# winddori2002/DEX-TTS

Measured on AMD Instinct MI355X. Metric: mel-frames/s at n_timesteps=50, 80-ch mel (sampler only); RTF, higher is better.
Workload: dtype bf16; 1 GPU; gedex_b1: gedex_lj B=1/GPU T=512 n_timesteps=50 (BASELINE.json configs[1]); global_batch=1, frames=512, hipgraph=False, parallelism=1 GPU

## Files before the change

dex_tts_amd/csrc/dex_api.hip:

```cpp
#include <hip/hip_runtime.h>
#include <cstdlib>

#include <cmath>
#include <cstdarg>
#include <atomic>
#include <cstdio>
#include <mutex>
#include <cstring>
#include <map>
#include <unordered_map>
#include <string_view>
#include <string>
#include <vector>

#include "../../include/dex_amd.h"
#include "kernels.h"
#include "weight_store.h"

using namespace dex;

namespace dex {
namespace {
const char* const KNOB_NAMES[] = {
    "DEX_CONV_STREAM", "DEX_CONV_PP", "DEX_CONV_SKIP_DEAD", "DEX_H_BF16", "DEX_ATTN_SEPARATE", "DEX_ATTN_Q64", "DEX_ATTN_Q64_TAIL", "DEX_ATTN_Q64_HALF", "DEX_DIT_XCDS", "DEX_ATTN_GENERIC", "DEX_RES2", "DEX_LP_INTER", "DEX_DIT_CHAIN",
    "DEX_DIT_CLUSTER", "DEX_DIT_CLUSTER_LOCAL", "DEX_ATTN_X_LP", "DEX_RES_X_LP", "DEX_CAT_LP", "DEX_XCD_MAP", "DEX_DEBUG_DROP_HANDOFF", "DEX_PATCH_FUSED",
    "DEX_CONV_DOWN", "DEX_CONVT_UP", "DEX_DEBUG_PLAN",
    "DEX_ATTN_SHARED_W8", "DEX_CONVT_MT", "DEX_CONVT_WGS", "DEX_CONV_DOWN_WGS", "DEX_CONV_REGW", "DEX_CONV_REGW_RES", "DEX_CONV_SMALL_MAX", "DEX_CONV_TH8",
    "DEX_CONV_W8", "DEX_DWCONV_CAP", "DEX_FINAL_CAP", "DEX_FIRST_CAP", "DEX_FIRST_MFMA", "DEX_GEMM_NWALK", "DEX_NWALK_SPLIT", "DEX_NWALK_BM", "DEX_POS_COL", "DEX_POS_COL_MIN",
    "DEX_POS_CT", "DEX_REGW_MIN_TILES", "DEX_REGW_WGS", "DEX_ROWCHAIN64", "DEX_ROWCHAIN64A", "DEX_TIV_CAP", "DEX_TV_CHAIN", "DEX_TIV_FOLD", "DEX_LINATTN_NSUB", "DEX_TV_FOLD", "DEX_OUT2_MIN", "DEX_NWALK_DMA",
    "DEX_LINATTN_HEADWAVES", "DEX_LINATTN_OUT2_HW", "DEX_CONV_ROUND1", "DEX_CONV_RESIDENT"};
constexpr int N_KNOBS = (int)(sizeof(KNOB_NAMES) / sizeof(KNOB_NAMES[0]));
int knob_parse(const char* e) {
    if (!e) return KNOB_UNSET;
    char* end = nullptr;
    const long v = strtol(e, &end, 10);
    if (end == e) {
        static bool warned = false;
        if (!warned) { warned = true; fprintf(stderr, "libdexamd: ignoring a DEX_* knob whose value '%s' is not an integer\n", e); }
        return KNOB_UNSET;
    }
// ... 1013 lines not shown
        DwConvP dw{};
        dw.X = X.p + X.coff; dw.ldx = X.ld; dw.xb = (long)P.Hm * P.Wm * X.ld; dw.Hi = P.Hm; dw.Wi = P.Wm; dw.C = mid;
        dw.k = c.dit_patch; dw.s = c.dit_stride; dw.pad = c.dit_patch / 2; dw.Wd = x->pe_dw; dw.bd = x->pe_db;
        dw.mask = mask_input ? mask : nullptr; dw.mask_ws = mask_ws; dw.mask_bstride = P.d.T;
        dw.Y = P.pe0; dw.Hf = P.Hf; dw.Wt = P.Wt; dw.B = B; dw.aff = in_aff;
        if (patch_fused()) {
            run("patch_embed", 2.0 * B * N * mid * (c.dit_patch * c.dit_patch + hid), 4.0 * B * (P.Hm * P.Wm * mid + N * hid),
                [&] { launch_patch_embed_fused(dw, x->pe_pw.nk[x->lpi()].p, x->pe_pb, P.emb, hid, x->precision, st); });
        } else {
            run("patch_dwconv_silu", 2.0 * B * N * mid * c.dit_patch * c.dit_patch, 4.0 * B * (P.Hm * P.Wm + N) * mid, [&] { launch_dwconv_silu(dw, st); });
            IGemmP pe = base_gemm(P.pe0, mid, 0, P.Hf, P.Wt, mid, x->pe_pw, hid, x->pe_pb, P.emb, hid, 0);
            gemm("patch_pointwise", pe);
        }
        const int G = c.dit_conv_pos_groups, kp = c.dit_conv_pos, cg = hid / G;
        int nsplit = POS_SPLIT, pcg = 0, pcgp = 0;
        if (x->lp() && x->pos_w.frag[x->lpi()].p) {
            PosConvP pcd{P.emb, x->pos_w.frag[x->lpi()].p, P.pos_part, P.Hf, P.Wt, hid, G, B};
            run("pos_conv", 2.0 * B * N * (double)kp * kp * cg * hid, 8.0 * B * N * hid + 2.0 * kp * kp * cg * hid, [&] { launch_pos_conv_direct(pcd, x->precision, st); });
            nsplit = 1;
        } else {
            const int cgp = (cg % 32) ? 64 : cg;
            const float* src = P.emb;
            if (cgp != cg) {
                run("pos_group_pad", 0, 8.0 * B * N * hid, [&] { launch_group_pad(P.emb, P.emb_pad, (long)B * N, G, cg, cgp, st); });
                src = P.emb_pad;
            }
            IGemmP pc = base_gemm(src, G * cgp, 0, P.Hf, P.Wt, cgp, x->pos_w, cgp, nullptr, P.pos_part, G * cgp, 0);
            pc.KH = kp; pc.KW = kp; pc.off_h = -(kp / 2); pc.off_w = -(kp / 2); pc.K = kp * kp * cgp;
            pc.groups = G; pc.w_gstride = (long)kp * kp * cgp * cgp; pc.ksplit = POS_SPLIT; pc.c_sstride = (long)B * N * G * cgp;
            gemm("pos_conv", pc);
            pcg = cgp != cg ? cg : 0; pcgp = cgp;
        }
        PosFinishP pf{P.pos_part, nsplit, (long)B * N * (pcg ? G * pcgp : hid), x->pos_b, P.emb, x->freq_pos, P.tok, P.Hf, P.Wt, hid, B, pcg, pcgp};
        run("pos_finish", 20.0 * B * N * hid, 4.0 * B * N * hid * (nsplit + 2), [&] { launch_pos_finish(pf, st); });
        if (debug) hipMemcpyAsync(P.dbg_tok, P.tok, (size_t)B * N * hid * 4, hipMemcpyDeviceToDevice, st);
        tap("tok_in", P.dbg_tok, (long)B * N, hid, hid);
        const float scale = 1.0f / sqrtf((float)(hid / c.dit_heads));
        const bool chain = x->lp() && dit_rowchain_supported(hid, mh) && c.dit_heads == 2 &&
                           !knob_off("DEX_DIT_CHAIN");
        for (int k = 0; k < c.dit_depth; ++k) {
            const DitBlockW& w = x->blocks[k];
            const float* ada = P.ada[k];
            const bool fuse_ln = x->lp() && ln_fusable(hid);
            DitChainP ch{};
            if (chain) {
                ch.ksplit = 0; ch.heads = c.dit_heads; ch.rows_per_batch = N; ch.X = P.tok; ch.ada = ada; ch.step = sp; ch.row_bstride = rbs; ch.M = B * N; ch.B = B;
                ch.Qh = (k & 1) ? P.qh : P.qh2; ch.Kh = (k & 1) ? P.kh : P.kh2; ch.Vt = (k & 1) ? P.vt : P.vt2;
                ch.Qin = (k & 1) ? P.qh2 : P.qh; ch.Kin = (k & 1) ? P.kh2 : P.kh; ch.Vin = (k & 1) ? P.vt2 : P.vt;
                ch.Npad = P.Npad;
// ... 100 lines not shown
                hipMemcpyAsync(dst, P.tok, (size_t)B * N * hid * 4, hipMemcpyDeviceToDevice, st);
                char nm[32]; snprintf(nm, sizeof nm, "tok_blk%d", k);
                tap(nm, dst, (long)B * N, hid, hid);
            }
        }
        const bool fuse_lnf = x->lp() && ln_fusable(hid);
        if (!fuse_lnf) {
            LnModP lf{P.tok, P.xn, N, hid, P.fin_mod, P.fin_mod + hid, 2L * hid, sp, B, rbs};
            run("ln_modulate", 8.0 * B * N * hid, 8.0 * B * N * hid, [&] { launch_ln_mod(lf, st); });
        }
        IGemmP fl = final_gemm(mask_ws, out, ldo, ocoff);
        if (cat_lp) { fl.C = reinterpret_cast<float*>(P.cat16); fl.c_lp = x->lp_kind(); }
        gemm("dit_final_unpatchify", fl);
    }

    bool patch_fused() const {
        const DexConfig& c = x->cfg;
        return x->lp() && !debug && !knob_off("DEX_PATCH_FUSED") &&
               patch_embed_fused_supported(c.dit_patch, mid_dim(c), c.dit_hidden, (long)P.d.B * P.N);
    }
    bool tiv_fold() const { return !debug && P.tiv_aff && knob_or("DEX_TIV_FOLD", 1) != 0; }
    bool tv_chain_on() const {
        return x->lp() && x->tv_wl.nk[x->lpi()].p && P.tv_kp && tv_chain_form(P.Hm * P.Wm, mid_dim(x->cfg), P.d.B);
    }
    bool tv_fold_on() const { return tv_chain_on() && x->lpi() != 2 && P.tv_G && knob_or("DEX_TV_FOLD", 1) != 0; }
    void dex_adaptors(const TD& X, int mask_ws) {
        const DexConfig& c = x->cfg;
        const int B = P.d.B, mid = mid_dim(c);
        const long npix = (long)P.Hm * P.Wm;
        InStatsP is{X.p + X.coff, X.ld, npix * X.ld, (int)npix, mid, P.tv_stats, B, mask, mask_ws, (long)P.d.T, P.Wm};
// ... 707 lines not shown
```

dex_tts_amd/csrc/kernels.h:

```cpp
#pragma once
#include <hip/hip_runtime.h>
#include <stdint.h>

namespace dex {

constexpr int KNOB_UNSET = -2147483647 - 1;
int knob(const char* name);
inline int knob_or(const char* name, int dflt) { const int v = knob(name); return v == KNOB_UNSET ? dflt : v; }
inline bool knob_off(const char* name) { return knob(name) == 0; }
inline bool knob_set(const char* name) { return knob(name) != KNOB_UNSET; }
inline int device_cus() {
    static const int n = [] { int dev = 0, v = 0; (void)hipGetDevice(&dev); (void)hipDeviceGetAttribute(&v, hipDeviceAttributeMultiprocessorCount, dev); return v > 0 ? v : 256; }();
    return n;
}

constexpr int GN_SLOTS = 32;
typedef long long gnfix_t;

extern thread_local const char* g_last_symbol;

constexpr int PREC_FP32 = 0, PREC_BF16 = 1, PREC_FP16 = 2, PREC_FP16X2 = 3;
inline bool prec_wsplit(int precision) { return precision == PREC_FP16X2; }
extern thread_local bool g_lp_wsplit;
inline bool prec_is_lp(int precision) { return precision != PREC_FP32; }
// ... 170 lines not shown
bool linattn_out2_lp_out_supported(int npix, int B);
bool linattn_fused_supported(int C);

struct DwConvP { const float* X; int ldx; long xb; int Hi, Wi, C; int k, s, pad; const float* Wd; const float* bd;
                 const float* mask; int mask_ws; long mask_bstride;
                 float* Y; int Hf, Wt; int B;
                 const float* aff = nullptr; };
void launch_dwconv_silu(const DwConvP& p, hipStream_t st);
bool patch_embed_fused_supported(int k, int C, int hid, long ntok);
void launch_patch_embed_fused(const DwConvP& p, const void* Wb, const float* bias, float* emb, int hid, int precision, hipStream_t st);

struct PosConvP { const float* X; const void* Wf; float* Y; int Hf, Wt, hid, G, B;
                  int ncol; };
bool pos_conv_direct_supported(int hid, int groups, int kernel, int Hf);
void launch_pos_conv_direct(const PosConvP& p, int precision, hipStream_t st);
struct PosFinishP { const float* part; int nsplit; long split_stride; const float* bias; const float* emb;
                    const float* freq_pos; float* tok; int Hf, Wt, D; int B;
                    int cg, cg_pad; };
void launch_pos_finish(const PosFinishP& p, hipStream_t st);
void launch_group_pad(const float* src, float* dst, long rows, int G, int cg, int cg_pad, hipStream_t st);

struct LnModP { const float* X; float* Y; int rows_per_batch; int D; const float* shift; const float* scale;
                long step_stride; int step; int B; int row_bstride = 0; };
void launch_ln_mod(const LnModP& p, hipStream_t st);

struct DitChainP { const float* O; int ksplit; long o_sstride; const float* ml; int heads; int rows_per_batch;
                   float* X; const void *Wp, *W1, *W2, *Wq; const float *bp, *b1, *b2, *bq;
                   const float* ada;
                   const float *next_shift, *next_scale; long next_step_stride;
                   void *Qh, *Kh, *Vt; int Npad; float qscale;
// ... 170 lines not shown
```

dex_tts_amd/csrc/kernels_lp.h:

```cpp
#include "kernels.h"
#include "lp_config.h"

namespace dex {
namespace DEX_LP_NS {

bool conv3x3_bf16_supported(int Cin, int Cout);
bool conv3x3_bf16_tail_supported(int C);
bool conv3x3_bf16_res_supported(int Cin, int Cout);
bool conv3x3_bf16_xb_supported(int Cin, int Cout);
void launch_conv3x3_lp(const Conv3P& p, hipStream_t st);
int conv3x3_stream_tiles(const Conv3P& p);
void launch_conv3x3_stream(const Conv3P& p, int tiles_per_wg, hipStream_t st);
bool conv3x3_regw_form(const Conv3P& p);
void launch_conv3x3_regw(const Conv3P& p, hipStream_t st);
bool linattn_out2_lp_out_supported(int npix, int B);
bool linattn_fused_supported(int C);
bool conv3x3_plain_lp_in_supported(int H, int W, int B, int Cin, int Cout);
bool conv3x3_res2_form(int H, int W, int B);
void launch_igemm_lp(const IGemmP& p, hipStream_t st);
bool attention_lp_shared_form(int Nq, int heads, int B, int ksplit);
bool igemm_nwalk_form(const IGemmP& p);
bool conv3x3_cat_lp_in_supported(int H, int W, int B, int Cin, int Cout);
bool convt_up_supported(int C, int H, int W, int ldx, int ldy);
void launch_convt_up(const ConvTUpP& p, hipStream_t st);
// ... 14 lines not shown
bool dit_rowchain_supported(int hidden, int mlp_hidden);
bool dit_rowchain64_form(int rows_per_batch, int B, int attn_inline);
bool dit_rowchain_cluster_form(int rows_per_batch, int B);
bool dit_rowchain_cluster_local_fits(int rows_per_batch, int B);
int dit_rowchain_cluster_xcds(int rows_per_batch, int B);
void launch_dit_rowchain(const DitChainP& p, hipStream_t st);
void launch_pack_lp_frag(const float* src, void* dst, int K, int N, hipStream_t st);
void launch_pack_lp_frag_nk(const float* src, void* dst, int K, int N, hipStream_t st);
void launch_linattn_kvctx(const LinKvCtxP& p, hipStream_t st);
void launch_linattn_merge(const LinMergeP& p, hipStream_t st);
void launch_linattn_out2(const LinOut2P& p, hipStream_t st);
bool patch_embed_fused_supported(int k, int C, int hid, long ntok);
void launch_patch_embed_fused(const DwConvP& p, const void* Wb, const float* bias, float* emb, int hid, hipStream_t st);
bool pos_conv_direct_supported(int hid, int groups, int kernel, int Hf);
void launch_pos_conv_direct(const PosConvP& p, hipStream_t st);

}
}
```

dex_tts_amd/csrc/lp_dispatch.hip:

```cpp
#include "kernels.h"

#include "kernels_lp.h"
#undef DEX_LP_NS
#define DEX_LP_NS f16
#include "kernels_lp.h"
#undef DEX_LP_NS
#define DEX_LP_NS f16w
#include "kernels_lp.h"
#undef DEX_LP_NS

namespace dex {

thread_local const char* g_last_symbol = nullptr;
thread_local bool g_lp_wsplit = false;

bool conv3x3_bf16_supported(int Cin, int Cout) { return (g_lp_wsplit ? f16w::conv3x3_bf16_supported(Cin, Cout) : bf16::conv3x3_bf16_supported(Cin, Cout)); }
bool conv3x3_bf16_tail_supported(int C) { return (g_lp_wsplit ? f16w::conv3x3_bf16_tail_supported(C) : bf16::conv3x3_bf16_tail_supported(C)); }
bool conv3x3_bf16_res_supported(int Cin, int Cout) { return (g_lp_wsplit ? f16w::conv3x3_bf16_res_supported(Cin, Cout) : bf16::conv3x3_bf16_res_supported(Cin, Cout)); }
bool conv3x3_bf16_xb_supported(int Cin, int Cout) { return (g_lp_wsplit ? f16w::conv3x3_bf16_xb_supported(Cin, Cout) : bf16::conv3x3_bf16_xb_supported(Cin, Cout)); }
bool conv3x3_plain_lp_in_supported(int H, int W, int B, int Cin, int Cout) { return (g_lp_wsplit ? f16w::conv3x3_plain_lp_in_supported(H, W, B, Cin, Cout) : bf16::conv3x3_plain_lp_in_supported(H, W, B, Cin, Cout)); }
bool linattn_out2_lp_out_supported(int npix, int B) { return (g_lp_wsplit ? f16w::linattn_out2_lp_out_supported(npix, B) : bf16::linattn_out2_lp_out_supported(npix, B)); }
bool linattn_fused_supported(int C) { return (g_lp_wsplit ? f16w::linattn_fused_supported(C) : bf16::linattn_fused_supported(C)); }
bool conv3x3_res2_form(int H, int W, int B) { return (g_lp_wsplit ? f16w::conv3x3_res2_form(H, W, B) : bf16::conv3x3_res2_form(H, W, B)); }
bool attention_lp_shared_form(int Nq, int heads, int B, int ksplit) { return (g_lp_wsplit ? f16w::attention_lp_shared_form(Nq, heads, B, ksplit) : bf16::attention_lp_shared_form(Nq, heads, B, ksplit)); }
bool igemm_nwalk_form(const IGemmP& p) { return (g_lp_wsplit ? f16w::igemm_nwalk_form(p) : bf16::igemm_nwalk_form(p)); }
bool conv3x3_cat_lp_in_supported(int H, int W, int B, int Cin, int Cout) { return (g_lp_wsplit ? f16w::conv3x3_cat_lp_in_supported(H, W, B, Cin, Cout) : bf16::conv3x3_cat_lp_in_supported(H, W, B, Cin, Cout)); }
bool conv3x3_strip_form(const Conv3P& p) { return (g_lp_wsplit ? f16w::conv3x3_stream_tiles(p) : bf16::conv3x3_stream_tiles(p)) != 0 || (g_lp_wsplit ? f16w::conv3x3_regw_form(p) : bf16::conv3x3_regw_form(p)); }
bool pos_conv_direct_supported(int hid, int groups, int kernel, int Hf) { return (g_lp_wsplit ? f16w::pos_conv_direct_supported(hid, groups, kernel, Hf) : bf16::pos_conv_direct_supported(hid, groups, kernel, Hf)); }
bool tv_chain_form(int npix, int C, int B) { return (g_lp_wsplit ? f16w::tv_chain_form(npix, C, B) : bf16::tv_chain_form(npix, C, B)); }
bool attention_direct_batch_regime(int N, int B) { return (g_lp_wsplit ? f16w::attention_direct_batch_regime(N, B) : bf16::attention_direct_batch_regime(N, B)); }
int attention_direct_ksplit(int N, int B) { return (g_lp_wsplit ? f16w::attention_direct_ksplit(N, B) : bf16::attention_direct_ksplit(N, B)); }
int attention_q64_ksplit(int N, int B, int max_split) { return (g_lp_wsplit ? f16w::attention_q64_ksplit(N, B, max_split) : bf16::attention_q64_ksplit(N, B, max_split)); }
void attention_q64_plan(int N, int B, int max_split, int* ks, int* tail_g, int* tail_ks) { (g_lp_wsplit ? f16w::attention_q64_plan(N, B, max_split, ks, tail_g, tail_ks) : bf16::attention_q64_plan(N, B, max_split, ks, tail_g, tail_ks)); }
bool conv_down_supported(int C, int H, int W, int ldx, int ldy, int x_coff) { return (g_lp_wsplit ? f16w::conv_down_supported(C, H, W, ldx, ldy, x_coff) : bf16::conv_down_supported(C, H, W, ldx, ldy, x_coff)); }
bool convt_up_supported(int C, int H, int W, int ldx, int ldy) { return (g_lp_wsplit ? f16w::convt_up_supported(C, H, W, ldx, ldy) : bf16::convt_up_supported(C, H, W, ldx, ldy)); }
bool patch_embed_fused_supported(int k, int C, int hid, long ntok) { return (g_lp_wsplit ? f16w::patch_embed_fused_supported(k, C, hid, ntok) : bf16::patch_embed_fused_supported(k, C, hid, ntok)); }
bool dit_rowchain_supported(int hidden, int mlp_hidden) { return (g_lp_wsplit ? f16w::dit_rowchain_supported(hidden, mlp_hidden) : bf16::dit_rowchain_supported(hidden, mlp_hidden)); }
bool dit_rowchain64_form(int rows_per_batch, int B, int attn_inline) { return (g_lp_wsplit ? f16w::dit_rowchain64_form(rows_per_batch, B, attn_inline) : bf16::dit_rowchain64_form(rows_per_batch, B, attn_inline)); }
bool dit_rowchain_cluster_form(int rows_per_batch, int B) { return (g_lp_wsplit ? f16w::dit_rowchain_cluster_form(rows_per_batch, B) : bf16::dit_rowchain_cluster_form(rows_per_batch, B)); }
int dit_rowchain_cluster_xcds(int rows_per_batch, int B) { return bf16::dit_rowchain_cluster_xcds(rows_per_batch, B); }
bool dit_rowchain_cluster_local_fits(int rows_per_batch, int B) { return (g_lp_wsplit ? f16w::dit_rowchain_cluster_local_fits(rows_per_batch, B) : bf16::dit_rowchain_cluster_local_fits(rows_per_batch, B)); }

#define DEX_LP_CALL(fn, ...) do { if (precision == PREC_FP16X2) f16w::fn(__VA_ARGS__); else if (precision == PREC_FP16) f16::fn(__VA_ARGS__); else bf16::fn(__VA_ARGS__); } while (0)
// ... 4 lines not shown
void launch_conv_down(const ConvDownP& p, int precision, hipStream_t st) { DEX_LP_CALL(launch_conv_down, p, st); }
void launch_attention_lp(const AttnP& p, int precision, hipStream_t st) { DEX_LP_CALL(launch_attention_lp, p, st); }
void launch_tv_kv_prep(const TvKvPrepP& p, int precision, hipStream_t st) { DEX_LP_CALL(launch_tv_kv_prep, p, st); }
void launch_tv_vfrag_prep(const TvKvPrepP& p, int precision, hipStream_t st) { DEX_LP_CALL(launch_tv_vfrag_prep, p, st); }
void launch_tv_chain(const TvChainP& p, int precision, hipStream_t st) { DEX_LP_CALL(launch_tv_chain, p, st); }
void launch_attention_direct(const AttnDirectP& p, int precision, hipStream_t st) { DEX_LP_CALL(launch_attention_direct, p, st); }
bool attention_q64_half_plan(int N, int B, int* half_g, int* half_n) { return bf16::attention_q64_half_plan(N, B, half_g, half_n); }
void launch_attention_q64(const AttnDirectP& p, int precision, hipStream_t st) { DEX_LP_CALL(launch_attention_q64, p, st); }
void launch_dit_rowchain(const DitChainP& p, int precision, hipStream_t st) { DEX_LP_CALL(launch_dit_rowchain, p, st); }
void launch_pack_lp_frag(const float* src, void* dst, int K, int N, int precision, hipStream_t st) { DEX_LP_CALL(launch_pack_lp_frag, src, dst, K, N, st); }
void launch_pack_lp_frag_nk(const float* src, void* dst, int K, int N, int precision, hipStream_t st) { DEX_LP_CALL(launch_pack_lp_frag_nk, src, dst, K, N, st); }
void launch_linattn_kvctx(const LinKvCtxP& p, int precision, hipStream_t st) { DEX_LP_CALL(launch_linattn_kvctx, p, st); }
void launch_linattn_merge(const LinMergeP& p, int precision, hipStream_t st) { DEX_LP_CALL(launch_linattn_merge, p, st); }
void launch_linattn_out2(const LinOut2P& p, int precision, hipStream_t st) { DEX_LP_CALL(launch_linattn_out2, p, st); }
void launch_pos_conv_direct(const PosConvP& p, int precision, hipStream_t st) { DEX_LP_CALL(launch_pos_conv_direct, p, st); }
void launch_patch_embed_fused(const DwConvP& p, const void* Wb, const float* bias, float* emb, int hid, int precision, hipStream_t st) { DEX_LP_CALL(launch_patch_embed_fused, p, Wb, bias, emb, hid, st); }

}
```

dex_tts_amd/csrc/patch_embed.hip:

```cpp
#include <hip/hip_runtime.h>
#include "kernels.h"
#include "lp_util.h"
#include "kernels_lp.h"

namespace dex {
namespace DEX_LP_NS {

typedef float f32x16 __attribute__((ext_vector_type(16)));
typedef unsigned short u16;

namespace {
constexpr int PE_TOK = 8;
__device__ __forceinline__ float silu_pe(float x) { return x * __builtin_amdgcn_rcpf(1.f + __expf(-x)); }
}

template <int KS, int C>
__global__ __launch_bounds__(256) void patch_embed_fused_kernel(const DwConvP p, const u16* __restrict__ Wb, const float* __restrict__ bias, float* __restrict__ emb, int hid) {
    constexpr int C4 = C / 4, LD = C + 8, KSTEPS = C / 16;
    constexpr int IPT = PE_TOK * C4 / 256;
    __shared__ __attribute__((aligned(16))) u16 As[32 * LD];
    const int tid = threadIdx.x, lane = tid & 63, wave = tid >> 6;
    const int i = lane & 31, hh = lane >> 5;
    const long ntok = (long)p.B * p.Hf * p.Wt;
    const long tok0 = (long)blockIdx.x * PE_TOK;
    const int ntile = hid / 32, per_wave = ntile / 4;
    union Fr { uint4 u; lp8 v; };
    Fr wf[2][KSTEPS];
#ifdef DEX_LP_WSPLIT
    Fr wl[2][KSTEPS];
#endif
    auto wload_tile = [&](int slot, int nt) __attribute__((always_inline)) {
        const u16* src = Wb + (long)(nt * 32 + i) * C + hh * 8;
#pragma unroll
        for (int ks = 0; ks < KSTEPS; ++ks) wf[slot][ks].u = *reinterpret_cast<const uint4*>(src + ks * 16);
    };
    auto wload_lo = [&](int slot, int nt) __attribute__((always_inline)) {
#ifdef DEX_LP_WSPLIT
        const u16* src = Wb + (long)hid * C + (long)(nt * 32 + i) * C + hh * 8;
#pragma unroll
        for (int ks = 0; ks < KSTEPS; ++ks) wl[slot][ks].u = *reinterpret_cast<const uint4*>(src + ks * 16);
#endif
    };
    wload_tile(0, wave * per_wave);
    if (per_wave > 1) wload_tile(1, wave * per_wave + 1);
    for (int q = tid; q < (32 - PE_TOK) * LD / 8; q += 256) *reinterpret_cast<uint4*>(As + PE_TOK * LD + q * 8) = make_uint4(0, 0, 0, 0);
    if (tid < PE_TOK * C4) {
        const int cq = tid % C4, tl = tid / C4;
        const long tok = min(tok0 + tl, ntok - 1);
        const int wt = (int)(tok % p.Wt);
        const int f = (int)((tok / p.Wt) % p.Hf);
        const int b = (int)(tok / ((long)p.Wt * p.Hf));
        const float* X = p.X + (long)b * p.xb;
        const float* mrow = p.mask ? p.mask + (long)b * p.mask_bstride : nullptr;
        float4 acc = *reinterpret_cast<const float4*>(p.bd + cq * 4);
        const float4 a4 = p.aff ? *reinterpret_cast<const float4*>(p.aff + ((long)b * 2 + 0) * p.C + cq * 4) : make_float4(1.f, 1.f, 1.f, 1.f);
        const float4 c4 = p.aff ? *reinterpret_cast<const float4*>(p.aff + ((long)b * 2 + 1) * p.C + cq * 4) : make_float4(0.f, 0.f, 0.f, 0.f);
#pragma unroll
        for (int kh = 0; kh < KS; ++kh) {
            const int hi = f * p.s + kh - p.pad;
#pragma unroll
// ... 4 lines not shown
                float4 v = *reinterpret_cast<const float4*>(X + ((long)hc * p.Wi + wc) * p.ldx + cq * 4);
                if (p.aff) { v.x = fmaf(v.x, a4.x, c4.x); v.y = fmaf(v.y, a4.y, c4.y); v.z = fmaf(v.z, a4.z, c4.z); v.w = fmaf(v.w, a4.w, c4.w); }
                const float4 w = *reinterpret_cast<const float4*>(p.Wd + (kh * KS + kw) * p.C + cq * 4);
                float mk = mrow ? mrow[wc * p.mask_ws] : 1.f;
                mk = inb ? mk : 0.f;
                acc.x = fmaf(v.x * mk, w.x, acc.x); acc.y = fmaf(v.y * mk, w.y, acc.y);
                acc.z = fmaf(v.z * mk, w.z, acc.z); acc.w = fmaf(v.w * mk, w.w, acc.w);
            }
        }
        uint2 o;
        o.x = pack2_lp(silu_pe(acc.x), silu_pe(acc.y)); o.y = pack2_lp(silu_pe(acc.z), silu_pe(acc.w));
        *reinterpret_cast<uint2*>(As + tl * LD + cq * 4) = o;
    }
    wload_lo(0, wave * per_wave);
    if (per_wave > 1) wload_lo(1, wave * per_wave + 1);
    __syncthreads();
    const u16* a_lane = As + i * LD + hh * 8;
    for (int t0 = 0; t0 < per_wave; t0 += 2) {
#pragma unroll
        for (int s_ = 0; s_ < 2; ++s_) {
            if (t0 + s_ >= per_wave) break;
            const int nt = wave * per_wave + t0 + s_;
            f32x16 acc;
#pragma unroll
            for (int r = 0; r < 16; ++r) acc[r] = 0.f;
#pragma unroll
            for (int ks = 0; ks < KSTEPS; ++ks) {
                const lp8 af = *reinterpret_cast<const lp8*>(a_lane + ks * 16);
                acc = DEX_MFMA_LP(af, wf[s_][ks].v, acc, 0, 0, 0);
#ifdef DEX_LP_WSPLIT
                acc = DEX_MFMA_LP(af, wl[s_][ks].v, acc, 0, 0, 0);
#endif
            }
            const float bv = bias ? bias[nt * 32 + i] : 0.f;
#pragma unroll
            for (int r = 0; r < 4; ++r) {
                const int rowl = r + 4 * hh;
                if (tok0 + rowl < ntok) emb[(tok0 + rowl) * hid + nt * 32 + i] = acc[r] + bv;
            }
        }
        if (t0 + 2 < per_wave) {
            wload_tile(0, wave * per_wave + t0 + 2); wload_lo(0, wave * per_wave + t0 + 2);
            if (t0 + 3 < per_wave) { wload_tile(1, wave * per_wave + t0 + 3); wload_lo(1, wave * per_wave + t0 + 3); }
        }
    }
}

bool patch_embed_fused_supported(int k, int C, int hid, long ntok) {
#if defined(DEX_LP_WSPLIT) && !defined(DEX_WS_HAVE_PE)
    return false;
#endif
   
    return (k == 3 || k == 7) && (C == 64 || C == 128) && hid % 128 == 0 && (ntok * (C / 4) + 255) / 256 < 320;
}

void launch_patch_embed_fused(const DwConvP& p, const void* Wb, const float* bias, float* emb, int hid, hipStream_t st) {
    const long ntok = (long)p.B * p.Hf * p.Wt;
    const dim3 grid((unsigned)((ntok + PE_TOK - 1) / PE_TOK));
    const u16* w = reinterpret_cast<const u16*>(Wb);
    g_last_symbol = "patch_embed_fused_kernel";
    if (p.k == 7 && p.C == 128) hipLaunchKernelGGL((patch_embed_fused_kernel<7, 128>), grid, dim3(256), 0, st, p, w, bias, emb, hid);
    else if (p.k == 7) hipLaunchKernelGGL((patch_embed_fused_kernel<7, 64>), grid, dim3(256), 0, st, p, w, bias, emb, hid);
    else if (p.C == 128) hipLaunchKernelGGL((patch_embed_fused_kernel<3, 128>), grid, dim3(256), 0, st, p, w, bias, emb, hid);
    else hipLaunchKernelGGL((patch_embed_fused_kernel<3, 64>), grid, dim3(256), 0, st, p, w, bias, emb, hid);
}

}
}
```

dex_tts_amd/csrc/pos_conv.hip:

```cpp
#include <hip/hip_runtime.h>
#include <cstdlib>
#include "kernels.h"
#include "lp_util.h"
#include "kernels_lp.h"

namespace dex {
namespace DEX_LP_NS {

typedef float f32x16 __attribute__((ext_vector_type(16)));
typedef unsigned u32x4 __attribute__((ext_vector_type(4)));
typedef unsigned short u16;

namespace {
constexpr int KP = 16, PAD = 8, CG = 32, LDP = CG;
}

template <int CT, bool COL>
__device__ __forceinline__ void pos_conv_body(const PosConvP& p, int rest) {
    constexpr int CW = 32 * CT, PW = CW + KP - 1;
    extern __shared__ __attribute__((aligned(16))) unsigned char smem_pc[];
    u16* patch = reinterpret_cast<u16*>(smem_pc);
    const int tid = threadIdx.x, lane = tid & 63, wave = tid >> 6;
    const int i = lane & 31, hh = lane >> 5;
    const int Hf = p.Hf, Wt = p.Wt;
// ... 122 lines not shown
            const float v = (red[((0 * CT + ct) * 32 + row) * 33 + n] + red[((1 * CT + ct) * 32 + row) * 33 + n]) +
                            (red[((2 * CT + ct) * 32 + row) * 33 + n] + red[((3 * CT + ct) * 32 + row) * 33 + n]);
            Y[(long)w * p.hid + n] = v;
        }
    }
}

template <int CT>
__global__ __launch_bounds__(256) void pos_conv_direct_kernel(const PosConvP p) {
    const int rest = blockIdx.x / p.G;
    const int nrow_wgs = ((p.Wt - p.ncol + 32 * CT - 1) / (32 * CT)) * p.Hf * p.B;
    if (rest >= nrow_wgs) pos_conv_body<CT, true>(p, rest);
    else pos_conv_body<CT, false>(p, rest);
}

bool pos_conv_direct_supported(int hid, int groups, int kernel, int Hf) {
#if defined(DEX_LP_WSPLIT) && !defined(DEX_WS_HAVE_POS)
    return false;
#endif
   
    return groups > 0 && hid / groups == CG && kernel == KP && Hf >= 1;
}

template <int CT>
static void launch_pc(const PosConvP& p, hipStream_t st) {
    constexpr int PW = 32 * CT + KP - 1;
    const int nrows = p.Hf < 2 * PAD ? p.Hf : 2 * PAD;
    size_t lds = (size_t)nrows * PW * LDP * sizeof(u16);
    const size_t lds_red = (size_t)4 * CT * 32 * 33 * sizeof(float);
    if (lds < lds_red) lds = lds_red;
    const size_t lds_col = p.ncol ? (size_t)(32 + 2 * PAD - 1) * (KP + 1) * LDP * sizeof(u16) : 0;
    if (lds < lds_col) lds = lds_col;
    static bool attr = false;
    if (!attr) {
        hipFuncSetAttribute(reinterpret_cast<const void*>(&pos_conv_direct_kernel<CT>), hipFuncAttributeMaxDynamicSharedMemorySize, 160 * 1024);
        attr = true;
// ... 29 lines not shown
```

Before: 28660 mel-frames/s.

## Fuse positional conv with GELU-mean pos_finish into column-chunk kernel

Adds a pos_conv_cols kernel in which each workgroup owns a group and a chunk of columns across all frequency rows. It computes the grouped 16x16 positional conv with MFMA, then applies bias, GELU, the mean over frequency, the residual add and freq_pos inside the same kernel, so the separate pos_finish launch and its partial-buffer round trip go away. It is chosen when the grid fits within the CU count. The diff also adds a token-granular patch-embed variant and cycle-counter timing stamps behind DEX_TIMING. The new kernel has a small grid and reloads the halo patch per column chunk, which could underuse the GPU.

```diff
diff --git a/dex_tts_amd/csrc/dex_api.hip b/dex_tts_amd/csrc/dex_api.hip
--- a/dex_tts_amd/csrc/dex_api.hip
+++ b/dex_tts_amd/csrc/dex_api.hip
@@ -23,7 +23,7 @@
 namespace {
 const char* const KNOB_NAMES[] = {
     "DEX_CONV_STREAM", "DEX_CONV_PP", "DEX_CONV_SKIP_DEAD", "DEX_H_BF16", "DEX_ATTN_SEPARATE", "DEX_ATTN_Q64", "DEX_ATTN_Q64_TAIL", "DEX_ATTN_Q64_HALF", "DEX_DIT_XCDS", "DEX_ATTN_GENERIC", "DEX_RES2", "DEX_LP_INTER", "DEX_DIT_CHAIN",
-    "DEX_DIT_CLUSTER", "DEX_DIT_CLUSTER_LOCAL", "DEX_ATTN_X_LP", "DEX_RES_X_LP", "DEX_CAT_LP", "DEX_XCD_MAP", "DEX_DEBUG_DROP_HANDOFF", "DEX_PATCH_FUSED",
+    "DEX_DIT_CLUSTER", "DEX_DIT_CLUSTER_LOCAL", "DEX_ATTN_X_LP", "DEX_RES_X_LP", "DEX_CAT_LP", "DEX_XCD_MAP", "DEX_DEBUG_DROP_HANDOFF", "DEX_PATCH_FUSED", "DEX_PATCH_TOK", "DEX_POS_FUSED", "DEX_POS_RING",
     "DEX_CONV_DOWN", "DEX_CONVT_UP", "DEX_DEBUG_PLAN",
     "DEX_ATTN_SHARED_W8", "DEX_CONVT_MT", "DEX_CONVT_WGS", "DEX_CONV_DOWN_WGS", "DEX_CONV_REGW", "DEX_CONV_REGW_RES", "DEX_CONV_SMALL_MAX", "DEX_CONV_TH8",
     "DEX_CONV_W8", "DEX_DWCONV_CAP", "DEX_FINAL_CAP", "DEX_FIRST_CAP", "DEX_FIRST_MFMA", "DEX_GEMM_NWALK", "DEX_NWALK_SPLIT", "DEX_NWALK_BM", "DEX_POS_COL", "DEX_POS_COL_MIN",
@@ -1067,7 +1067,12 @@
         }
         const int G = c.dit_conv_pos_groups, kp = c.dit_conv_pos, cg = hid / G;
         int nsplit = POS_SPLIT, pcg = 0, pcgp = 0;
-        if (x->lp() && x->pos_w.frag[x->lpi()].p) {
+        if (x->lp() && x->pos_w.frag[x->lpi()].p && pos_cols(G, kp)) {
+            PosColsP pcc{P.emb, x->pos_w.frag[x->lpi()].p, x->pos_b, x->freq_pos, P.tok, P.Hf, P.Wt, hid, G, B};
+            run("pos_conv_tail", 2.0 * B * N * (double)kp * kp * cg * hid + 20.0 * B * N * hid, 12.0 * B * N * hid + 2.0 * kp * kp * cg * hid,
+                [&] { launch_pos_conv_cols(pcc, x->precision, st); });
+            nsplit = 0;
+        } else if (x->lp() && x->pos_w.frag[x->lpi()].p) {
             PosConvP pcd{P.emb, x->pos_w.frag[x->lpi()].p, P.pos_part, P.Hf, P.Wt, hid, G, B};
             run("pos_conv", 2.0 * B * N * (double)kp * kp * cg * hid, 8.0 * B * N * hid + 2.0 * kp * kp * cg * hid, [&] { launch_pos_conv_direct(pcd, x->precision, st); });
             nsplit = 1;
@@ -1084,8 +1089,10 @@
             gemm("pos_conv", pc);
             pcg = cgp != cg ? cg : 0; pcgp = cgp;
         }
-        PosFinishP pf{P.pos_part, nsplit, (long)B * N * (pcg ? G * pcgp : hid), x->pos_b, P.emb, x->freq_pos, P.tok, P.Hf, P.Wt, hid, B, pcg, pcgp};
-        run("pos_finish", 20.0 * B * N * hid, 4.0 * B * N * hid * (nsplit + 2), [&] { launch_pos_finish(pf, st); });
+        if (nsplit) {
+            PosFinishP pf{P.pos_part, nsplit, (long)B * N * (pcg ? G * pcgp : hid), x->pos_b, P.emb, x->freq_pos, P.tok, P.Hf, P.Wt, hid, B, pcg, pcgp};
+            run("pos_finish", 20.0 * B * N * hid, 4.0 * B * N * hid * (nsplit + 2), [&] { launch_pos_finish(pf, st); });
+        }
         if (debug) hipMemcpyAsync(P.dbg_tok, P.tok, (size_t)B * N * hid * 4, hipMemcpyDeviceToDevice, st);
         tap("tok_in", P.dbg_tok, (long)B * N, hid, hid);
         const float scale = 1.0f / sqrtf((float)(hid / c.dit_heads));
@@ -1216,6 +1223,11 @@
         gemm("dit_final_unpatchify", fl);
     }
 
+    bool pos_cols(int G, int kp) const {
+        const DexConfig& c = x->cfg;
+        if (debug || knob_off("DEX_POS_FUSED") || !pos_conv_cols_supported(c.dit_hidden, G, kp, P.Hf, P.Wt, P.d.B)) return false;
+        return knob_or("DEX_POS_FUSED", 0) == 1 || pos_conv_cols_grid(G, P.Hf, P.Wt, P.d.B) <= device_cus();
+    }
     bool patch_fused() const {
         const DexConfig& c = x->cfg;
         return x->lp() && !debug && !knob_off("DEX_PATCH_FUSED") &&
diff --git a/dex_tts_amd/csrc/kernels.h b/dex_tts_amd/csrc/kernels.h
--- a/dex_tts_amd/csrc/kernels.h
+++ b/dex_tts_amd/csrc/kernels.h
@@ -208,6 +208,11 @@
                   int ncol; };
 bool pos_conv_direct_supported(int hid, int groups, int kernel, int Hf);
 void launch_pos_conv_direct(const PosConvP& p, int precision, hipStream_t st);
+struct PosColsP { const float* X; const void* Wf; const float* bias; const float* freq_pos; float* tok; int Hf, Wt, hid, G, B;
+                  int ncols, pw; };
+bool pos_conv_cols_supported(int hid, int groups, int kernel, int Hf, int Wt, int B);
+long pos_conv_cols_grid(int groups, int Hf, int Wt, int B);
+void launch_pos_conv_cols(const PosColsP& p, int precision, hipStream_t st);
 struct PosFinishP { const float* part; int nsplit; long split_stride; const float* bias; const float* emb;
                     const float* freq_pos; float* tok; int Hf, Wt, D; int B;
                     int cg, cg_pad; };
diff --git a/dex_tts_amd/csrc/kernels_lp.h b/dex_tts_amd/csrc/kernels_lp.h
--- a/dex_tts_amd/csrc/kernels_lp.h
+++ b/dex_tts_amd/csrc/kernels_lp.h
@@ -52,6 +52,9 @@
 void launch_patch_embed_fused(const DwConvP& p, const void* Wb, const float* bias, float* emb, int hid, hipStream_t st);
 bool pos_conv_direct_supported(int hid, int groups, int kernel, int Hf);
 void launch_pos_conv_direct(const PosConvP& p, hipStream_t st);
+bool pos_conv_cols_supported(int hid, int groups, int kernel, int Hf, int Wt, int B);
+long pos_conv_cols_grid(int groups, int Hf, int Wt, int B);
+void launch_pos_conv_cols(const PosColsP& p, hipStream_t st);
 
 }
 }
diff --git a/dex_tts_amd/csrc/lp_dispatch.hip b/dex_tts_amd/csrc/lp_dispatch.hip
--- a/dex_tts_amd/csrc/lp_dispatch.hip
+++ b/dex_tts_amd/csrc/lp_dispatch.hip
@@ -27,6 +27,8 @@
 bool conv3x3_cat_lp_in_supported(int H, int W, int B, int Cin, int Cout) { return (g_lp_wsplit ? f16w::conv3x3_cat_lp_in_supported(H, W, B, Cin, Cout) : bf16::conv3x3_cat_lp_in_supported(H, W, B, Cin, Cout)); }
 bool conv3x3_strip_form(const Conv3P& p) { return (g_lp_wsplit ? f16w::conv3x3_stream_tiles(p) : bf16::conv3x3_stream_tiles(p)) != 0 || (g_lp_wsplit ? f16w::conv3x3_regw_form(p) : bf16::conv3x3_regw_form(p)); }
 bool pos_conv_direct_supported(int hid, int groups, int kernel, int Hf) { return (g_lp_wsplit ? f16w::pos_conv_direct_supported(hid, groups, kernel, Hf) : bf16::pos_conv_direct_supported(hid, groups, kernel, Hf)); }
+bool pos_conv_cols_supported(int hid, int groups, int kernel, int Hf, int Wt, int B) { return (g_lp_wsplit ? f16w::pos_conv_cols_supported(hid, groups, kernel, Hf, Wt, B) : bf16::pos_conv_cols_supported(hid, groups, kernel, Hf, Wt, B)); }
+long pos_conv_cols_grid(int groups, int Hf, int Wt, int B) { return bf16::pos_conv_cols_grid(groups, Hf, Wt, B); }
 bool tv_chain_form(int npix, int C, int B) { return (g_lp_wsplit ? f16w::tv_chain_form(npix, C, B) : bf16::tv_chain_form(npix, C, B)); }
 bool attention_direct_batch_regime(int N, int B) { return (g_lp_wsplit ? f16w::attention_direct_batch_regime(N, B) : bf16::attention_direct_batch_regime(N, B)); }
 int attention_direct_ksplit(int N, int B) { return (g_lp_wsplit ? f16w::attention_direct_ksplit(N, B) : bf16::attention_direct_ksplit(N, B)); }
@@ -61,6 +63,7 @@
 void launch_linattn_merge(const LinMergeP& p, int precision, hipStream_t st) { DEX_LP_CALL(launch_linattn_merge, p, st); }
 void launch_linattn_out2(const LinOut2P& p, int precision, hipStream_t st) { DEX_LP_CALL(launch_linattn_out2, p, st); }
 void launch_pos_conv_direct(const PosConvP& p, int precision, hipStream_t st) { DEX_LP_CALL(launch_pos_conv_direct, p, st); }
+void launch_pos_conv_cols(const PosColsP& p, int precision, hipStream_t st) { DEX_LP_CALL(launch_pos_conv_cols, p, st); }
 void launch_patch_embed_fused(const DwConvP& p, const void* Wb, const float* bias, float* emb, int hid, int precision, hipStream_t st) { DEX_LP_CALL(launch_patch_embed_fused, p, Wb, bias, emb, hid, st); }
 
 }
diff --git a/dex_tts_amd/csrc/patch_embed.hip b/dex_tts_amd/csrc/patch_embed.hip
--- a/dex_tts_amd/csrc/patch_embed.hip
+++ b/dex_tts_amd/csrc/patch_embed.hip
@@ -14,8 +14,29 @@
 __device__ __forceinline__ float silu_pe(float x) { return x * __builtin_amdgcn_rcpf(1.f + __expf(-x)); }
 }
 
+#ifdef DEX_TIMING
+long long* g_pe_dbg = nullptr;
+#define PE_DBG_PARAM , long long* dbg
+#define PE_DBG_ARG , g_pe_dbg
+#define PSTAMP_DECL long long tk[8] = {0, 0, 0, 0, 0, 0, 0, 0}; const long long tk0 = __builtin_readcyclecounter(); long long tlast = tk0;
+#define PSTAMP(k) do { const long long now_ = __builtin_readcyclecounter(); tk[k] += now_ - tlast; tlast = now_; } while (0)
+#define PSTAMP_STORE(n)                                                                     \
+    if (dbg && threadIdx.x == 0) {                                                          \
+        long long* d_ = dbg + (long)blockIdx.x * 8;                                         \
+        for (int k_ = 0; k_ < (n); ++k_) d_[k_] = tk[k_];                                   \
+        d_[7] = __builtin_readcyclecounter() - tk0;                                         \
+    }
+#else
+#define PE_DBG_PARAM
+#define PE_DBG_ARG
+#define PSTAMP_DECL
+#define PSTAMP(k) do {} while (0)
+#define PSTAMP_STORE(n)
+#endif
+
 template <int KS, int C>
-__global__ __launch_bounds__(256) void patch_embed_fused_kernel(const DwConvP p, const u16* __restrict__ Wb, const float* __restrict__ bias, float* __restrict__ emb, int hid) {
+__global__ __launch_bounds__(256) void patch_embed_fused_kernel(const DwConvP p, const u16* __restrict__ Wb, const float* __restrict__ bias, float* __restrict__ emb, int hid PE_DBG_PARAM) {
+    PSTAMP_DECL
     constexpr int C4 = C / 4, LD = C + 8, KSTEPS = C / 16;
     constexpr int IPT = PE_TOK * C4 / 256;
     __shared__ __attribute__((aligned(16))) u16 As[32 * LD];
@@ -44,6 +65,7 @@
     wload_tile(0, wave * per_wave);
     if (per_wave > 1) wload_tile(1, wave * per_wave + 1);
     for (int q = tid; q < (32 - PE_TOK) * LD / 8; q += 256) *reinterpret_cast<uint4*>(As + PE_TOK * LD + q * 8) = make_uint4(0, 0, 0, 0);
+    PSTAMP(0);
     if (tid < PE_TOK * C4) {
         const int cq = tid % C4, tl = tid / C4;
         const long tok = min(tok0 + tl, ntok - 1);
@@ -78,7 +100,9 @@
     }
     wload_lo(0, wave * per_wave);
     if (per_wave > 1) wload_lo(1, wave * per_wave + 1);
+    PSTAMP(2);
     __syncthreads();
+    PSTAMP(3);
     const u16* a_lane = As + i * LD + hh * 8;
     for (int t0 = 0; t0 < per_wave; t0 += 2) {
 #pragma unroll
@@ -97,17 +121,158 @@
 #endif
             }
             const float bv = bias ? bias[nt * 32 + i] : 0.f;
+            PSTAMP(4);
 #pragma unroll
             for (int r = 0; r < 4; ++r) {
                 const int rowl = r + 4 * hh;
                 if (tok0 + rowl < ntok) emb[(tok0 + rowl) * hid + nt * 32 + i] = acc[r] + bv;
             }
+            PSTAMP(5);
         }
         if (t0 + 2 < per_wave) {
             wload_tile(0, wave * per_wave + t0 + 2); wload_lo(0, wave * per_wave + t0 + 2);
             if (t0 + 3 < per_wave) { wload_tile(1, wave * per_wave + t0 + 3); wload_lo(1, wave * per_wave + t0 + 3); }
         }
     }
+    PSTAMP_STORE(6)
+}
+
+template <int KS, int C, int TOK>
+__global__ __launch_bounds__(256) void patch_embed_fused_tok_kernel(const DwConvP p, const u16* __restrict__ Wb, const float* __restrict__ bias, float* __restrict__ emb, int hid PE_DBG_PARAM) {
+    PSTAMP_DECL
+    constexpr int V = TOK * C > 256 ? 2 : 1, CV = C / V, LD = C + 8, KSTEPS = C / 16;
+    static_assert(TOK >= 1 && TOK <= 4 && TOK * CV <= 256, "one item per thread");
+    constexpr int NWQ = KS * KS * C / 4, WPT = (NWQ + 255) / 256;
+    __shared__ __attribute__((aligned(16))) u16 As[32 * LD];
+    __shared__ __attribute__((aligned(16))) float Wds[KS * KS * C];
+    const int tid = threadIdx.x, lane = tid & 63, wave = tid >> 6;
+    const int i = lane & 31, hh = lane >> 5;
+    const long ntok = (long)p.B * p.Hf * p.Wt;
+    const long tok0 = (long)blockIdx.x * TOK;
+    const int ntile = hid / 32, per_wave = ntile / 4;
+    union Fr { uint4 u; lp8 v; };
+    Fr wf[2][KSTEPS];
+#ifdef DEX_LP_WSPLIT
+    Fr wl[2][KSTEPS];
+#endif
+    auto wload_tile = [&](int slot, int nt) __attribute__((always_inline)) {
+        const u16* src = Wb + (long)(nt * 32 + i) * C + hh * 8;
+#pragma unroll
+        for (int ks = 0; ks < KSTEPS; ++ks) wf[slot][ks].u = *reinterpret_cast<const uint4*>(src + ks * 16);
+    };
+    auto wload_lo = [&](int slot, int nt) __attribute__((always_inline)) {
+#ifdef DEX_LP_WSPLIT
+        const u16* src = Wb + (long)hid * C + (long)(nt * 32 + i) * C + hh * 8;
+#pragma unroll
+        for (int ks = 0; ks < KSTEPS; ++ks) wl[slot][ks].u = *reinterpret_cast<const uint4*>(src + ks * 16);
+#endif
+    };
+    wload_tile(0, wave * per_wave);
+    if (per_wave > 1) wload_tile(1, wave * per_wave + 1);
+    float4 wst[WPT];
+#pragma unroll
+    for (int q = 0; q < WPT; ++q) wst[q] = *reinterpret_cast<const float4*>(p.Wd + (long)min(tid + 256 * q, NWQ - 1) * 4);
+    const bool act = tid < TOK * CV;
+    const int cv = tid % CV, tl = tid / CV;
+    const long tok = min(tok0 + tl, ntok - 1);
+    const int wt = (int)(tok % p.Wt);
+    const int f = (int)((tok / p.Wt) % p.Hf);
+    const int b = (int)(tok / ((long)p.Wt * p.Hf));
+    float xv[KS * KS][V], cmk[KS], acc[V], a_[V], c_[V];
+    if (act) {
+        const float* X = p.X + (long)b * p.xb + cv * V;
+        const float* mrow = p.mask ? p.mask + (long)b * p.mask_bstride : nullptr;
+#pragma unroll
+        for (int kw = 0; kw < KS; ++kw) {
+            const int wi = wt * p.s + kw - p.pad;
+            cmk[kw] = mrow ? mrow[((unsigned)wi < (unsigned)p.Wi ? wi : 0) * p.mask_ws] : 1.f;
+        }
+#pragma unroll
+        for (int j = 0; j < V; ++j) {
+            acc[j] = p.bd[cv * V + j];
+            a_[j] = p.aff ? p.aff[((long)b * 2 + 0) * p.C + cv * V + j] : 1.f;
+            c_[j] = p.aff ? p.aff[((long)b * 2 + 1) * p.C + cv * V + j] : 0.f;
+        }
+#pragma unroll
+        for (int kh = 0; kh < KS; ++kh) {
+            const int hi = f * p.s + kh - p.pad;
+#pragma unroll
+            for (int kw = 0; kw < KS; ++kw) {
+                const int wi = wt * p.s + kw - p.pad;
+                const bool inb = (unsigned)hi < (unsigned)p.Hi && (unsigned)wi < (unsigned)p.Wi;
+                const int hc = inb ? hi : 0, wc = inb ? wi : 0;
+                const float* src = X + ((long)hc * p.Wi + wc) * p.ldx;
+                if (V == 2) { const float2 v = *reinterpret_cast<const float2*>(src); xv[kh * KS + kw][0] = v.x; xv[kh * KS + kw][V - 1] = v.y; }
+                else xv[kh * KS + kw][0] = *src;
+            }
+        }
+    }
+    PSTAMP(0);
+#pragma unroll
+    for (int q = 0; q < WPT; ++q)
+        if (tid + 256 * q < NWQ) *reinterpret_cast<float4*>(Wds + (tid + 256 * q) * 4) = wst[q];
+    for (int q = tid; q < (32 - TOK) * LD / 8; q += 256) *reinterpret_cast<uint4*>(As + TOK * LD + q * 8) = make_uint4(0, 0, 0, 0);
+    __syncthreads();
+    PSTAMP(1);
+    if (act) {
+#pragma unroll
+        for (int kh = 0; kh < KS; ++kh) {
+            const int hi = f * p.s + kh - p.pad;
+#pragma unroll
+            for (int kw = 0; kw < KS; ++kw) {
+                const int wi = wt * p.s + kw - p.pad;
+                const bool inb = (unsigned)hi < (unsigned)p.Hi && (unsigned)wi < (unsigned)p.Wi;
+                const float mk = inb ? cmk[kw] : 0.f;
+                const float* wsrc = Wds + (kh * KS + kw) * C + cv * V;
+                float w[V];
+                if (V == 2) { const float2 w2 = *reinterpret_cast<const float2*>(wsrc); w[0] = w2.x; w[V - 1] = w2.y; }
+                else w[0] = *wsrc;
+#pragma unroll
+                for (int j = 0; j < V; ++j) {
+                    float v = xv[kh * KS + kw][j];
+                    if (p.aff) v = fmaf(v, a_[j], c_[j]);
+                    acc[j] = fmaf(v * mk, w[j], acc[j]);
+                }
+            }
+        }
+        if (V == 2) *reinterpret_cast<unsigned*>(As + tl * LD + cv * V) = pack2_lp(silu_pe(acc[0]), silu_pe(acc[V - 1]));
+        else As[tl * LD + cv] = (u16)(pack2_lp_asm(silu_pe(acc[0]), 0.f) & 0xffffu);
+    }
+    wload_lo(0, wave * per_wave);
+    if (per_wave > 1) wload_lo(1, wave * per_wave + 1);
+    PSTAMP(2);
+    __syncthreads();
+    PSTAMP(3);
+    const u16* a_lane = As + i * LD + hh * 8;
+    for (int t0 = 0; t0 < per_wave; t0 += 2) {
+#pragma unroll
+        for (int s_ = 0; s_ < 2; ++s_) {
+            if (t0 + s_ >= per_wave) break;
+            const int nt = wave * per_wave + t0 + s_;
+            f32x16 ac;
+#pragma unroll
+            for (int r = 0; r < 16; ++r) ac[r] = 0.f;
+#pragma unroll
+            for (int ks = 0; ks < KSTEPS; ++ks) {
+                const lp8 af = *reinterpret_cast<const lp8*>(a_lane + ks * 16);
+                ac = DEX_MFMA_LP(af, wf[s_][ks].v, ac, 0, 0, 0);
+#ifdef DEX_LP_WSPLIT
+                ac = DEX_MFMA_LP(af, wl[s_][ks].v, ac, 0, 0, 0);
+#endif
+            }
+            const float bv = bias ? bias[nt * 32 + i] : 0.f;
+            PSTAMP(4);
+#pragma unroll
+            for (int r = 0; r < TOK; ++r)
+                if (hh == 0 && tok0 + r < ntok) emb[(tok0 + r) * hid + nt * 32 + i] = ac[r] + bv;
+            PSTAMP(5);
+        }
+        if (t0 + 2 < per_wave) {
+            wload_tile(0, wave * per_wave + t0 + 2); wload_lo(0, wave * per_wave + t0 + 2);
+            if (t0 + 3 < per_wave) { wload_tile(1, wave * per_wave + t0 + 3); wload_lo(1, wave * per_wave + t0 + 3); }
+        }
+    }
+    PSTAMP_STORE(6)
 }
 
 bool patch_embed_fused_supported(int k, int C, int hid, long ntok) {
@@ -118,16 +283,33 @@
     return (k == 3 || k == 7) && (C == 64 || C == 128) && hid % 128 == 0 && (ntok * (C / 4) + 255) / 256 < 320;
 }
 
+static int patch_tok(long ntok) {
+    const int k = knob_or("DEX_PATCH_TOK", 0);
+    if (k == 2 || k == 3 || k == 4 || k == 8) return k;
+    for (int t = 3; t <= 4; ++t)
+        if ((ntok + t - 1) / t <= device_cus()) return t;
+    return PE_TOK;
+}
+
+template <int KS, int C>
+static void launch_pe(int tok, dim3 block, const DwConvP& p, const u16* w, const float* bias, float* emb, int hid, hipStream_t st) {
+    const long ntok = (long)p.B * p.Hf * p.Wt;
+    const dim3 grid((unsigned)((ntok + tok - 1) / tok));
+    if (tok == 2) { g_last_symbol = "patch_embed_fused_tok_kernel<2>"; hipLaunchKernelGGL((patch_embed_fused_tok_kernel<KS, C, 2>), grid, block, 0, st, p, w, bias, emb, hid PE_DBG_ARG); }
+    else if (tok == 3) { g_last_symbol = "patch_embed_fused_tok_kernel<3>"; hipLaunchKernelGGL((patch_embed_fused_tok_kernel<KS, C, 3>), grid, block, 0, st, p, w, bias, emb, hid PE_DBG_ARG); }
+    else if (tok == 4) { g_last_symbol = "patch_embed_fused_tok_kernel<4>"; hipLaunchKernelGGL((patch_embed_fused_tok_kernel<KS, C, 4>), grid, block, 0, st, p, w, bias, emb, hid PE_DBG_ARG); }
+    else { g_last_symbol = "patch_embed_fused_kernel"; hipLaunchKernelGGL((patch_embed_fused_kernel<KS, C>), grid, block, 0, st, p, w, bias, emb, hid PE_DBG_ARG); }
+}
+
 void launch_patch_embed_fused(const DwConvP& p, const void* Wb, const float* bias, float* emb, int hid, hipStream_t st) {
     const long ntok = (long)p.B * p.Hf * p.Wt;
-    const dim3 grid((unsigned)((ntok + PE_TOK - 1) / PE_TOK));
+    const int tok = patch_tok(ntok);
     const u16* w = reinterpret_cast<const u16*>(Wb);
-    g_last_symbol = "patch_embed_fused_kernel";
-    if (p.k == 7 && p.C == 128) hipLaunchKernelGGL((patch_embed_fused_kernel<7, 128>), grid, dim3(256), 0, st, p, w, bias, emb, hid);
-    else if (p.k == 7) hipLaunchKernelGGL((patch_embed_fused_kernel<7, 64>), grid, dim3(256), 0, st, p, w, bias, emb, hid);
-    else if (p.C == 128) hipLaunchKernelGGL((patch_embed_fused_kernel<3, 128>), grid, dim3(256), 0, st, p, w, bias, emb, hid);
-    else hipLaunchKernelGGL((patch_embed_fused_kernel<3, 64>), grid, dim3(256), 0, st, p, w, bias, emb, hid);
-}
-
-}
-}
+    if (p.k == 7 && p.C == 128) launch_pe<7, 128>(tok, dim3(256), p, w, bias, emb, hid, st);
+    else if (p.k == 7) launch_pe<7, 64>(tok, dim3(256), p, w, bias, emb, hid, st);
+    else if (p.C == 128) launch_pe<3, 128>(tok, dim3(256), p, w, bias, emb, hid, st);
+    else launch_pe<3, 64>(tok, dim3(256), p, w, bias, emb, hid, st);
+}
+
+}
+}
diff --git a/dex_tts_amd/csrc/pos_conv.hip b/dex_tts_amd/csrc/pos_conv.hip
--- a/dex_tts_amd/csrc/pos_conv.hip
+++ b/dex_tts_amd/csrc/pos_conv.hip
@@ -160,12 +160,190 @@
     else pos_conv_body<CT, false>(p, rest);
 }
 
+template <int RING>
+__global__ __launch_bounds__(256) void pos_conv_cols_kernel(const PosColsP p) {
+    extern __shared__ __attribute__((aligned(16))) unsigned char smem_pc[];
+    u16* patch = reinterpret_cast<u16*>(smem_pc);
+    const int tid = threadIdx.x, lane = tid & 63, wave = tid >> 6;
+    const int i = lane & 31, hh = lane >> 5;
+    const int Hf = p.Hf, Wt = p.Wt, ncols = p.ncols, pw = p.pw;
+    const int nchunk = (Wt + ncols - 1) / ncols;
+    const int g = blockIdx.x % p.G;
+    const int rest = blockIdx.x / p.G;
+    const int w0 = (rest % nchunk) * ncols, b = rest / nchunk;
+    const int nrows = Hf + 2 * PAD - 1;
+    constexpr int NT = KP * KP;
+
+    const u32x4* Wf = reinterpret_cast<const u32x4*>(p.Wf) + (long)g * (NT * 2 * 64) + lane;
+    u32x4 wr[RING][2];
+#ifdef DEX_LP_WSPLIT
+    u32x4 wl[RING][2];
+    const long lo_u4 = (long)p.G * (NT * 2 * 64);
+#define PC_LOAD_LO(d, tap) do { wl[d][0] = Wf[lo_u4 + ((tap) * 2 + 0) * 64]; wl[d][1] = Wf[lo_u4 + ((tap) * 2 + 1) * 64]; } while (0)
+#else
+#define PC_LOAD_LO(d, tap) do { } while (0)
+#endif
+#pragma unroll
+    for (int d = 0; d < RING; ++d) {
+        const int t = wave + 4 * d;
+        wr[d][0] = Wf[(t * 2 + 0) * 64];
+        wr[d][1] = Wf[(t * 2 + 1) * 64];
+        PC_LOAD_LO(d, t);
+    }
+    {
+        const float* X = p.X + ((long)b * Hf * Wt) * p.hid + g * CG;
+        const int items = nrows * pw * 4;
+        for (int it0 = 0; it0 < items; it0 += 256 * 9) {
+            float4 f0[9], f1[9];
+            bool ok[9];
+#pragma unroll
+            for (int q = 0; q < 9; ++q) {
+                const int it = min(it0 + tid + 256 * q, items - 1);
+                const int c8 = (it & 3) * 8, px = it >> 2;
+                const int pc = px % pw, pr = px / pw;
+                const int wi = w0 + pc - PAD, hi = pr - PAD;
+                ok[q] = (unsigned)wi < (unsigned)Wt && (unsigned)hi < (unsigned)Hf;
+                const float* src = X + ((long)(ok[q] ? hi : 0) * Wt + (ok[q] ? wi : 0)) * p.hid + c8;
+                f0[q] = *reinterpret_cast<const float4*>(src);
+                f1[q] = *reinterpret_cast<const float4*>(src + 4);
+            }
+#pragma unroll
+            for (int q = 0; q < 9; ++q) {
+                const int it = it0 + tid + 256 * q;
+                if (it < items) {
+                    const float m = ok[q] ? 1.f : 0.f;
+                    uint4 v;
+                    v.x = pack2_lp(f0[q].x * m, f0[q].y * m); v.y = pack2_lp(f0[q].z * m, f0[q].w * m);
+                    v.z = pack2_lp(f1[q].x * m, f1[q].y * m); v.w = pack2_lp(f1[q].z * m, f1[q].w * m);
+                    const int px = it >> 2;
+                    *reinterpret_cast<uint4*>(patch + px * LDP + (((it & 3) ^ ((px >> 2) & 3)) * 8)) = v;
+                }
+            }
+        }
+    }
+    f32x16 acc;
+#pragma unroll
+    for (int r = 0; r < 16; ++r) acc[r] = 0.f;
+    lds_barrier();
+
+    const int live = Hf * ncols;
+    const int li = min(i, live - 1);
+    const int px0 = (li / ncols) * pw + li % ncols;
+    for (int n0 = 0; n0 < NT / 4; n0 += RING) {
+#pragma unroll
+        for (int d = 0; d < RING; ++d) {
+            const int t = wave + 4 * (n0 + d);
+            const int px = px0 + (t >> 4) * pw + (t & 15);
+            const int sw = (px >> 2) & 3;
+            const u16* ap = patch + (long)px * LDP;
+            const lp8 a0 = *reinterpret_cast<const lp8*>(ap + ((hh ^ sw) * 8));
+            const lp8 a1 = *reinterpret_cast<const lp8*>(ap + (((2 + hh) ^ sw) * 8));
+            acc = DEX_MFMA_LP(a0, __builtin_bit_cast(lp8, wr[d][0]), acc, 0, 0, 0);
+            acc = DEX_MFMA_LP(a1, __builtin_bit_cast(lp8, wr[d][1]), acc, 0, 0, 0);
+#ifdef DEX_LP_WSPLIT
+            acc = DEX_MFMA_LP(a0, __builtin_bit_cast(lp8, wl[d][0]), acc, 0, 0, 0);
+            acc = DEX_MFMA_LP(a1, __builtin_bit_cast(lp8, wl[d][1]), acc, 0, 0, 0);
+#endif
+            const int tn = min(t + 4 * RING, NT - 4 + wave);
+            wr[d][0] = Wf[(tn * 2 + 0) * 64];
+            wr[d][1] = Wf[(tn * 2 + 1) * 64];
+            PC_LOAD_LO(d, tn);
+        }
+    }
+#undef PC_LOAD_LO
+    lds_barrier();
+    float* red = reinterpret_cast<float*>(smem_pc);
+    float* part = red + 4 * 32 * 33;
+#pragma unroll
+    for (int r = 0; r < 16; ++r) red[(wave * 32 + (r & 3) + 8 * (r >> 2) + 4 * hh) * 33 + i] = acc[r];
+    lds_barrier();
+    {
+#pragma clang fp contract(off)
+        const int nitem = ncols * 128;
+        for (int idx = tid; idx < nitem; idx += 256) {
+            const int n = idx & 31, fl = (idx >> 5) & 3, c = idx >> 7;
+            const float bias = p.bias[g * CG + n];
+            float ps = 0.f;
+            for (int f = fl; f < Hf; f += 4) {
+                const int row = f * ncols + c;
+                const float v = (red[(0 * 32 + row) * 33 + n] + red[(1 * 32 + row) * 33 + n]) + (red[(2 * 32 + row) * 33 + n] + red[(3 * 32 + row) * 33 + n]);
+                const float a = bias + v;
+                ps = fmaf(0.5f * a, 1.0f + erff(a * 0.70710678118654752440f), ps);
+            }
+            part[(fl * ncols + c) * 32 + n] = ps;
+        }
+        lds_barrier();
+        const float inv = 1.f / (float)Hf;
+        for (int idx = tid; idx < nitem; idx += 256) {
+            const int n = idx & 31, fl = (idx >> 5) & 3, c = idx >> 7;
+            const int w = w0 + c;
+            if (w >= Wt) continue;
+            const float pos = (((part[(0 * ncols + c) * 32 + n] + part[(1 * ncols + c) * 32 + n]) + part[(2 * ncols + c) * 32 + n]) + part[(3 * ncols + c) * 32 + n]) * inv;
+            for (int f = fl; f < Hf; f += 4) {
+                const long o = (((long)b * Hf + f) * Wt + w) * p.hid + g * CG + n;
+                const float e = p.X[o];
+                const float fp = p.freq_pos[(long)f * p.hid + g * CG + n];
+                p.tok[o] = (e + pos) + fp;
+            }
+        }
+    }
+}
+
 bool pos_conv_direct_supported(int hid, int groups, int kernel, int Hf) {
 #if defined(DEX_LP_WSPLIT) && !defined(DEX_WS_HAVE_POS)
     return false;
 #endif
    
     return groups > 0 && hid / groups == CG && kernel == KP && Hf >= 1;
+}
+
+static int pos_conv_ncol(int Hf, int Wt, int B, int G) {
+    const bool col_off = knob_off("DEX_POS_COL");
+    const long col_min = knob_or("DEX_POS_COL_MIN", 512);
+    return (!col_off && Wt > 32 && Wt % 32 == 1 && Hf <= 32 && (long)Hf * B * G >= col_min) ? 1 : 0;
+}
+bool pos_conv_cols_supported(int hid, int groups, int kernel, int Hf, int Wt, int B) {
+    return pos_conv_direct_supported(hid, groups, kernel, Hf) && Hf >= 1 && 32 / Hf >= 2 && pos_conv_ncol(Hf, Wt, B, groups) == 0;
+}
+long pos_conv_cols_grid(int groups, int Hf, int Wt, int B) {
+    const int ncols = 32 / Hf;
+    return (long)((Wt + ncols - 1) / ncols) * B * groups;
+}
+
+void launch_pos_conv_cols(const PosColsP& p0, hipStream_t st) {
+    PosColsP p = p0;
+    p.ncols = 32 / p.Hf;
+    const int live = p.Hf * p.ncols;
+    int best = 0, best_worst = 1 << 30;
+    for (int pw = p.ncols + KP - 1; pw < p.ncols + KP - 1 + 16 && best_worst > 1; ++pw) {
+        int worst = 0;
+        for (int grp = 0; grp < 2; ++grp) {
+            int cnt[16] = {0}, seen[32] = {0};
+            for (int l = 0; l < 32; ++l) {
+                const bool g0 = l < 4 || (l >= 12 && l < 16) || (l >= 20 && l < 28);
+                const int li = l < live ? l : live - 1;
+                if (g0 != (grp == 0) || seen[li]) continue;
+                seen[li] = 1;
+                const int m = ++cnt[((li / p.ncols) * pw + li % p.ncols) & 15];
+                if (m > worst) worst = m;
+            }
+        }
+        if (worst < best_worst) { best_worst = worst; best = pw; }
+    }
+    p.pw = best;
+    size_t lds = (size_t)(p.Hf + 2 * PAD - 1) * p.pw * LDP * sizeof(u16);
+    const size_t lds_red = (size_t)(4 * 32 * 33 + 4 * p.ncols * 32) * sizeof(float);
+    if (lds < lds_red) lds = lds_red;
+#ifdef DEX_LP_WSPLIT
+    const int ring = 8;
+#else
+    const int ring = knob_or("DEX_POS_RING", 8) == 16 ? 16 : 8;
+#endif
+    const dim3 grid((unsigned)pos_conv_cols_grid(p.G, p.Hf, p.Wt, p.B));
+    if (ring == 8) { g_last_symbol = "pos_conv_cols_kernel<8>"; hipLaunchKernelGGL(pos_conv_cols_kernel<8>, grid, dim3(256), lds, st, p); }
+#ifndef DEX_LP_WSPLIT
+    else { g_last_symbol = "pos_conv_cols_kernel<16>"; hipLaunchKernelGGL(pos_conv_cols_kernel<16>, grid, dim3(256), lds, st, p); }
+#endif
 }
 
 template <int CT>
```

Result: faster. 29120 mel-frames/s (median of 6 runs) (+1.6%).
